# meco-group/omg-tools

Measured on AMD Instinct MI355X. Metric: MPC solves/sec, 1024-agent Holonomic Point2point batch per GPU, higher is better.
Workload: dtype f64

## Files before the change

include/omgx.h:

```cpp
#ifndef OMGX_H
#define OMGX_H
#include <stdint.h>

#ifdef __cplusplus
extern "C" {
#endif

#define OMGX_VERSION 9
#define OMGX_TERM_VARS 4

#define OMGX_OK            0
#define OMGX_E_INVALID    -1
#define OMGX_E_NODEVICE   -2
#define OMGX_E_HIP        -3
#define OMGX_E_TOOLARGE   -4

#define OMGX_SOLVE_SUCCEEDED        0
#define OMGX_MAX_ITER_EXCEEDED      1
#define OMGX_INFEASIBLE_DETECTED    2
#define OMGX_UNSUPPORTED_BOUNDS     3
#define OMGX_NUMERICAL_FAILURE      4

#define OMGX_PTR_DEVICE     1
#define OMGX_BOUNDS_SHARED  2
// ... 71 lines not shown
int  omgx_template_read(const char* path, omgx_template** out);
void omgx_template_free(omgx_template* tpl);

int  omgx_version(void);
const char* omgx_last_error(void);
const char* omgx_status_string(int32_t status);
void omgx_default_options(omgx_options* o);

int  omgx_template_n_blocks(const omgx_template* tpl, int32_t kind);
int  omgx_template_block_at(const omgx_template* tpl, int32_t kind, int32_t i, const char** name, int32_t* off,
                            int32_t* rows, int32_t* cols);
int  omgx_template_block(const omgx_template* tpl, int32_t kind, const char* name, int32_t* off, int32_t* rows,
                         int32_t* cols);

int  omgx_plan_describe(const omgx_template* tpl, omgx_plan_info* info, int32_t* order);

int  omgx_batch_create(const omgx_template* tpl, int32_t n_agents, int32_t device,
                       omgx_batch** out);
void omgx_batch_destroy(omgx_batch* b);
int  omgx_batch_set_options(omgx_batch* b, const omgx_options* o);
int  omgx_batch_set_stream(omgx_batch* b, void* hip_stream);
int  omgx_batch_set_order(omgx_batch* b, const int32_t* order_device);
int  omgx_batch_order_by_iters(omgx_batch* b, const int32_t* iters_device, int32_t* order_device);
int  omgx_batch_set_restarts(omgx_batch* b, const double* x0_alt_device, int32_t n_alt, int32_t* attempts_device);
int  omgx_batch_lds_bytes(const omgx_batch* b);
#define OMGX_HAS_LAST_INSTANCE 1
int  omgx_batch_last_instance(const omgx_batch* b);
int  omgx_batch_workspace(const omgx_batch* b, int32_t* mode, int64_t* lds_bytes,
                          int64_t* hbm_bytes_per_slab, int32_t* n_slabs);

// ... 194 lines not shown
```

omg-tools_amd/csrc/omgx.hip:

```cpp
#include <hip/hip_runtime.h>
#include <hip/hip_ext.h>
#include <cmath>
#include <stdarg.h>
#include <stdio.h>
#include <stdlib.h>
#include <string.h>
#include <string>
#include <vector>
#include "../../include/omgx.h"
#include "omgx_core.h"
#include "omgx_plan.h"
#include "omgx_kernels.h"
#include "omgx_table_cache.h"

namespace {

thread_local std::string g_err;

#define HIPCHK(call)                                                              \
  do {                                                                            \
    hipError_t e_ = (call);                                                       \
    if (e_ != hipSuccess) {                                                       \
      g_err = std::string(#call) + ": " + hipGetErrorString(e_);                  \
      return OMGX_E_HIP;                                                          \
// ... 405 lines not shown
  memset(info, 0, sizeof *info);
  info->n_leaf = d.n_leaf; info->n_root = d.n_root; info->n_eq = d.n_eq; info->nnz_j = d.nnz_j;
  info->kkt_doubles = plan.kkt_doubles; info->wave_path = d.wave_ok;
  info->ws_mode = mode;
  info->lds_bytes = (int64_t)(nl * sizeof(double));
  for (int l = 0; l < d.n_leaf && l < OMGX_PLAN_MAX_LEAF; ++l) {
    info->leaf_size[l] = plan.leaf_off[l + 1] - plan.leaf_off[l];
    info->leaf_bw[l] = plan.leaf_bw[l];
    info->leaf_cpl[l] = plan.cpl_ptr[l + 1] - plan.cpl_ptr[l];
  }
  info->n_pairs = d.n_pairs; info->ka_len = d.ka_len; info->kh_len = d.kh_len; info->kg_len = d.kg_len;
  if (order) for (int q = 0; q < d.N; ++q) order[q] = plan.order[q];
  return OMGX_OK;
}

namespace {
struct TplField { int kind; size_t count; const void* const* src; void** dst; };

size_t tpl_fields(const omgx_template& t, omgx_template* m, TplField* f, int term_vars = OMGX_TERM_VARS) {
  const omgx_template& s = t;
  size_t k = 0;
#define OMGX_F(KD, NAME, CNT) f[k].kind = KD; f[k].count = (size_t)(CNT); f[k].src = (const void* const*)&s.NAME; f[k].dst = m ? (void**)&m->NAME : nullptr; ++k;
  OMGX_F(0, prog, 6 * (size_t)t.n_prog)      OMGX_F(1, knots, t.n_knots)       OMGX_F(0, pp_ptr, t.n_pp + 1)
  OMGX_F(1, pm_coef, t.n_mono)               OMGX_F(0, pm_ptr, t.n_mono + 1)   OMGX_F(0, pm_atom, t.n_matom)
  OMGX_F(0, slot_pp, t.n_slots)              OMGX_F(0, row_ptr, t.n_con + 2)   OMGX_F(1, t_coef, t.n_terms)
  OMGX_F(0, t_slot, t.n_terms)               OMGX_F(0, t_var, (size_t)term_vars * t.n_terms)
  OMGX_F(0, eq_rows, t.n_eq)                 OMGX_F(0, root_vars, t.n_root_vars)
  OMGX_F(2, block_names, t.block_names_len)  OMGX_F(0, block_kind, t.n_blocks)        OMGX_F(0, block_off, t.n_blocks)
  OMGX_F(0, block_rows, t.n_blocks)          OMGX_F(0, block_cols, t.n_blocks)
  OMGX_F(1, lbg_def, t.has_bounds ? t.n_con : 0)  OMGX_F(1, ubg_def, t.has_bounds ? t.n_con : 0)
// ... 1314 lines not shown
```

omg-tools_amd/csrc/omgx_core.h:

```cpp
#pragma once
#include <stdint.h>
#include <math.h>

#ifdef OMGX_HOST_PORT
#define OMGX_FN inline
#define OMGX_HD inline
#define OMGX_HDF inline
#else
#define OMGX_FN __device__ __forceinline__
#define OMGX_HD __host__ __device__ inline
#define OMGX_HDF __host__ __device__ __forceinline__
#endif

#ifdef OMGX_HOST_PORT
#include <vector>
static thread_local std::vector<double> omgx_rbak;
#endif
#ifdef OMGX_COUNT_FACT
#include <atomic>
static std::atomic<long> omgx_dbg_nfact(0);
static std::atomic<long> omgx_dbg_cnt[12];
#endif
namespace omgx {

// ... 18 lines not shown
  int general;
  int rp_packed;
  int n_knots;
  int atoms_alias;
  int wave_ok;
  int n_jv;
  int n_jv4, n_ja4;
  int ka_len, kh_len, kg_len;
  int n_kafix, n_kgfix;
  int n_khfix;
  int side_off, dump_off;
  int n_cs_own;
  int kg_side_dinv;
  int n_owner;
  int n_lift, lift_depth;
};

struct MonoRec { double coef; int16_t a0, a1, a2, a3; };
struct MonoRec8 { double coef; int16_t a0, a1, a2, a3, a4, a5, a6, a7; };

#define OMGX_TV 4
struct JItem { double coef; int16_t slot, va, vb, vc; };
struct RowTerm { double coef; int32_t slot; int16_t v0, v1, v2, v3; };
struct HItem { double coef; int32_t row, target; int16_t slot, vthird, vfourth, kind; };

struct Tables {
  const int32_t* prog; const double* knots;
  const int32_t* pp_ptr; const double* pm_coef; const int32_t* pm_ptr; const int32_t* pm_atom;
  const int32_t* slot_pp;
  const MonoRec* pm_rec;
// ... 301 lines not shown
    if (kHbm) { __builtin_amdgcn_fence(__ATOMIC_RELEASE, "workgroup"); __builtin_amdgcn_wave_barrier(); __builtin_amdgcn_fence(__ATOMIC_ACQUIRE, "workgroup"); }
    else { __builtin_amdgcn_fence(__ATOMIC_RELEASE, "wavefront"); __builtin_amdgcn_wave_barrier(); __builtin_amdgcn_fence(__ATOMIC_ACQUIRE, "wavefront"); }
  }
};
typedef CtxT<false> Ctx;
#endif

#define OMGX_PFOR(i, n) for (int i = c.tid(); i < (n); i += c.nthr())
#define OMGX_PFOR_U4(i, n) _Pragma("unroll 4") for (int i = c.tid(); i < (n); i += c.nthr())

enum { PH_JAC = 0, PH_RESID, PH_ASSEMBLE, PH_FACTOR, PH_SOLVE, PH_STEP, PH_LINESEARCH, PH_UPDATE, PH_F_LEAF, PH_F_SCHUR, PH_F_ROOT, PH_LA, PH_LS, PH_LB, PH_SETUP, PH_TOTAL,
       PH_S_DESC, PH_S_PARAMS, PH_S_JAC0, PH_S_CLASS, PH_S_INIT, PH_A_ZERO, PH_A_PAIRS, PH_A_REST, PH_A_DIAG,
       PH_K_FWD, PH_K_ROOTRHS, PH_K_ROOT, PH_K_LEAFRHS, PH_K_BWD, PH_L_TERMS, PH_L_ROWS,
       PH_F_PARK, PH_F_SWEEP, PH_F_SCALE, PH_A_TCOL, PH_A_HESS, PH_P_LOAD, PH_P_DIV, PH_P_BSPL, PH_P_SLOTS,
       PH_WG_HEAD, PH_WG_TAIL,
       PH_COUNT };
#if defined(OMGX_PROFILE) && !defined(OMGX_HOST_PORT)
#define OMGX_TIC() long long tic_ = (c.sync(), clock64())
#define OMGX_TOC(k) do { c.sync(); long long now_ = clock64(); if (c.tid() == 0 && c.prof) c.prof[k] += now_ - tic_; tic_ = now_; } while (0)
#else
#define OMGX_TIC() do {} while (0)
#define OMGX_TOC(k) do {} while (0)
#endif

OMGX_FN double pp_eval(const Tables& T, int pp, const double* a) {
  double tot = 0.0;
  for (int m = T.pp_ptr[pp]; m < T.pp_ptr[pp + 1]; ++m) {
    double v = T.pm_coef[m];
    for (int q = T.pm_ptr[m]; q < T.pm_ptr[m + 1]; ++q) v *= a[T.pm_atom[q]];
    tot += v;
// ... 698 lines not shown
  Mr.a = ROOT_LDS ? 0 : K.d_off[d.n_leaf]; Mr.ld = 0; Mr.nfact = d.nr; Mr.rows = d.nr + 1; Mr.npos = d.n_root; Mr.dinv = -1; Mr.pan = pan0; Mr.cpl = 0; Mr.bw = d.nr;
  Mr.pad_ = K.d_off[d.n_leaf];
}

template <class C>
OMGX_FN void kkt_describe(const C& c, const Dims& d, const Kkt& K, Work& w, bool sync_after = true) {
  const int who = c.nthr() > 64 ? 64 : 0;
  if (c.tid() == who) kkt_describe_fill<C::wave_only, C::hbm, C::root_lds>(d, K, (BMat*)w.col);
  if (sync_after) c.sync();
}

template <class C>
OMGX_FN void kkt_descriptors(const C& c, const Dims& d, const Tables& T, Work& w, bool sync_after = true) {
  if constexpr (C::wave_only) {
    const int t0 = c.nthr() > 64 ? 64 : 0, nt = c.nthr() > 64 ? 64 : c.nthr();
    const int i0 = c.tid() - t0, n = (d.n_leaf + 1) * (int)(sizeof(BMat) / sizeof(int32_t));
    int32_t* Ms = (int32_t*)w.col;
    if (i0 >= 0 && i0 < nt) for (int i = i0; i < n; i += nt) Ms[i] = T.bmat_img[i];
    if (sync_after) c.sync();
  } else {
    Kkt K; K.bind(d, T, w.kkt);
    kkt_describe(c, d, K, w, sync_after);
  }
}

#ifndef OMGX_HOST_PORT
OMGX_FN WPanel wpanel_leaf(const BMat& M) {
  WPanel P; P.base = M.a; P.ld = M.ld; P.n = M.nfact; P.nreg = M.rows - 2; P.nvec = 2; P.npos = M.nfact; P.bw = M.bw;
  P.vrow = M.rows - 2; P.band = M.bw; P.ldb = M.pad_; P.wbase = M.pan;
  return P;
}
OMGX_FN WPanel wpanel_root(const BMat& M, int n_root) {
  WPanel P; P.base = M.a; P.ld = 0; P.n = M.nfact; P.nreg = M.nfact; P.nvec = 1; P.npos = n_root; P.bw = M.nfact;
  P.vrow = M.nfact; P.band = -1; P.ldb = 0; P.wbase = 0;
  return P;
}

struct DiagLeaf { int base, n, S, dinv, dl; };
OMGX_FN DiagLeaf diag_leaf(const BMat& M) {
  DiagLeaf L;
  L.base = __builtin_amdgcn_readfirstlane(M.a); L.n = __builtin_amdgcn_readfirstlane(M.nfact);
  L.S = __builtin_amdgcn_readfirstlane(M.pan); L.dinv = __builtin_amdgcn_readfirstlane(M.dinv); L.dl = 4 * L.dinv;
  return L;
}

template <class C>
OMGX_FN int kkt_factor_wave(const C& c, const Dims& d, const Kkt& K, Work& w) {
  typedef double v4d __attribute__((ext_vector_type(4)));
  const BMat* Ms = (const BMat*)w.col;
  const int lane = c.lane(), wave = c.wave(), nw = c.nwaves();
  const int koff = (int)(w.kkt - omgx_lds);
  OMGX_TIC();
  int badl = 0;
#ifdef OMGX_PROFILE
  const long long tw0_ = clock64();
#endif
  for (int l = wave; l < d.n_leaf; l += nw) {
    const int kind_bw = __builtin_amdgcn_readfirstlane(Ms[l].bw);
    if (kind_bw < 0) {
      const DiagLeaf L = diag_leaf(Ms[l]);
      const double dj = w.kkt[L.base + (lane < L.n ? lane : 0)];
      if (lane < L.n) { w.dinv[L.dinv + lane] = rcp_pivot(dj); if (!(dj > 0.0)) badl = 1; }
      continue;
    }
    const WPanel P = wpanel_leaf(Ms[l]);
    const int leaf_n = __builtin_amdgcn_readfirstlane(Ms[l].nfact);
    if (wave_leaf_small(leaf_n, kind_bw)) badl |= wave_ldl<OMGX_LEAF_COLS_SMALL, OMGX_LEAF_BW_SMALL, true, 2>(koff, P);
    else badl |= (kind_bw <= 8) ? wave_ldl<OMGX_WAVE_COLS, 8, true, 2>(koff, P) : wave_ldl<OMGX_WAVE_COLS, OMGX_WAVE_COLS, true, 2>(koff, P);
    wave_fence();
    const double dl = wave_dinv<true>(w.kkt, P);
    if (lane < P.n) w.dinv[Ms[l].dinv + lane] = dl;
  }
#ifdef OMGX_PROFILE
  if (c.tid() == 0) { c.prof[PH_F_SCALE] += clock64() - tw0_; c.prof[PH_F_PARK] += 1; }
#endif
  if (c.rmax(badl ? 1.0 : 0.0) > 0.0) return 1;
  OMGX_TOC(PH_F_LEAF);
  double* R = K.R();
  for (int base = 0; base < d.n_leaf; base += nw) {
    const int l = base + wave;
    v4d acc00 = {0.0, 0.0, 0.0, 0.0}, acc10 = acc00, acc11 = acc00;
    int nc1 = 0, ci_b0 = 0, ci_b1 = 0, ci_a[8];
    bool sparse = false;
#pragma unroll
    for (int i = 0; i < 8; ++i) ci_a[i] = 0;
    if (l < d.n_leaf) {
      const BMat M = Ms[l];
      sparse = __builtin_amdgcn_readfirstlane(M.bw) < 0;
      if (!sparse) {
      const int n = __builtin_amdgcn_readfirstlane(M.nfact), ld = __builtin_amdgcn_readfirstlane(M.ld);
      nc1 = __builtin_amdgcn_readfirstlane(M.rows) - n;
      const double* Wt = w.kkt + __builtin_amdgcn_readfirstlane(M.pan);
      const double* di = w.dinv + __builtin_amdgcn_readfirstlane(M.dinv);
      const int32_t* ci = K.cpl_idx + __builtin_amdgcn_readfirstlane(M.cpl);
      const int cb0 = lane & 15, cb1 = 16 + (lane & 15);
      ci_b0 = ci[cb0 < nc1 - 1 ? cb0 : 0]; ci_b1 = ci[cb1 < nc1 - 1 ? cb1 : 0];
#pragma unroll
      for (int i = 0; i < 8; ++i) {
        const int ca = 16 * (i >> 2) + (lane >> 4) + 4 * (i & 3);
        ci_a[i] = ca < nc1 - 1 ? ci[ca] : d.nr;
      }
      const int r0 = lane & 15, r1 = 16 + (lane & 15), q = lane >> 4;
      const int r0c = r0 < nc1 ? r0 : nc1 - 1, r1c = r1 < nc1 ? r1 : nc1 - 1;
      const bool two = nc1 > 16;
      for (int j0 = 0; j0 < n; j0 += 4) {
        const int j = j0 + q, jc = j < n ? j : n - 1;
        const double w0 = Wt[r0c * ld + jc], w1 = Wt[r1c * ld + jc], dj = di[jc];
        const double b0 = (r0 < nc1 && j < n) ? w0 : 0.0, b1 = (r1 < nc1 && j < n) ? w1 : 0.0;
        acc00 = __builtin_amdgcn_mfma_f64_16x16x4f64(b0 * dj, b0, acc00, 0, 0, 0);
        if (two) {
          acc10 = __builtin_amdgcn_mfma_f64_16x16x4f64(b1 * dj, b0, acc10, 0, 0, 0);
          acc11 = __builtin_amdgcn_mfma_f64_16x16x4f64(b1 * dj, b1, acc11, 0, 0, 0);
        }
      }
      }
    }
    const int lend = base + nw < d.n_leaf ? base + nw : d.n_leaf;
    for (int lr = base; lr < lend; ++lr) {
      if (l == lr && !sparse) {
        const int cb0 = lane & 15, cb1 = 16 + (lane & 15);
#pragma unroll
        for (int i = 0; i < 4; ++i) {
          const int ca0 = (lane >> 4) + 4 * i, ca1 = 16 + ca0;
          if (ca0 < nc1 && cb0 < nc1 - 1 && cb0 <= ca0) R[tri(ci_a[i], ci_b0)] -= acc00[i];
          if (ca1 < nc1 && cb0 < nc1 - 1) R[tri(ci_a[4 + i], ci_b0)] -= acc10[i];
          if (ca1 < nc1 && cb1 < nc1 - 1 && cb1 <= ca1) R[tri(ci_a[4 + i], ci_b1)] -= acc11[i];
        }
      } else if (l == lr) {
        const DiagLeaf L = diag_leaf(Ms[l]);
        const int j = lane < L.n ? lane : 0;
        const bool on = lane < L.n;
        const double* A = w.kkt + L.base + j;
        const double di = w.dinv[L.dinv + j];
        const double vt = A[(1 + L.S) * L.n], rj = A[(2 + L.S) * L.n];
        const int pt = d.n_root - 1;
        double vs[4]; int ps[4];
#pragma unroll
        for (int s = 0; s < 4; ++s) {
          const bool has = s < L.S;
          ps[s] = has ? K.dl_pos[L.dl + s * L.n + j] : -1;
          const double v = A[(1 + (has ? s : 0)) * L.n];
          vs[s] = (has && on && ps[s] >= 0) ? v : 0.0;
        }
        if (on) {
#pragma unroll
          for (int s = 0; s < 4; ++s) {
            if (ps[s] < 0 || s >= L.S) continue;
            const double u = vs[s] * di;
#pragma unroll
            for (int s2 = 0; s2 <= s; ++s2) {
              if (ps[s2] < 0) continue;
              const int pa = ps[s] > ps[s2] ? ps[s] : ps[s2], pb = ps[s] > ps[s2] ? ps[s2] : ps[s];
              R[tri(pa, pb)] -= u * vs[s2];
            }
            R[tri(pt, ps[s])] -= u * vt;
            R[tri(d.nr, ps[s])] -= u * rj;
          }
        }
        const double stt = c.wave_sum(on ? vt * di * vt : 0.0), srt = c.wave_sum(on ? rj * di * vt : 0.0);
        if (lane == 0) { R[tri(pt, pt)] -= stt; R[tri(d.nr, pt)] -= srt; }
      }
      c.sync();
    }
  }
  OMGX_TOC(PH_F_SCHUR);
  int badr = 0;
  if (wave == 0) {
    const WPanel P = wpanel_root(Ms[d.n_leaf], d.n_root);
#ifdef OMGX_PROFILE
    const long long tr0_ = clock64();
#endif
    badr = wave_ldl<OMGX_WAVE_COLS, OMGX_WAVE_COLS, false, 1>(koff, P);
#ifdef OMGX_PROFILE
    if (c.tid() == 0) c.prof[PH_F_SWEEP] += clock64() - tr0_;
#endif
  }
  const int bad = c.rmax(badr ? 1.0 : 0.0) > 0.0 ? 2 : 0;
  OMGX_TOC(PH_F_ROOT);
  return bad;
}
// ... 22 lines not shown
    const double y = w.kkt[wcarried<false>(P, P.n) + (lane < P.n ? lane : 0)];
    const double x = wave_bwd<OMGX_WAVE_COLS, false>(koff, P, dl, y * dl);
    if (lane < P.n) sol[d.root_off + lane] = x;
  }
  c.sync();
  OMGX_TOC(PH_K_ROOT);
  double* xg = w.col + OMGX_BMAT_DOUBLES * (OMGX_MAX_LEAF + 1) + wave * 64;
  for (int l = wave; l < d.n_leaf; l += nw) {
    const BMat M = Ms[l];
    if (__builtin_amdgcn_readfirstlane(M.bw) < 0) {
      const DiagLeaf L = diag_leaf(M);
      const int j = lane < L.n ? lane : 0;
      const double* A = w.kkt + L.base + j;
      double acc = A[(2 + L.S) * L.n] - A[(1 + L.S) * L.n] * sol[d.root_off + d.n_root - 1];
      for (int s = 0; s < L.S; ++s) {
        const int ps = K.dl_pos[L.dl + s * L.n + j];
        acc = fma(-A[(1 + s) * L.n], sol[d.root_off + (ps < 0 ? 0 : ps)] * (ps < 0 ? 0.0 : 1.0), acc);
      }
      if (lane < L.n) sol[L.dinv + lane] = acc * w.dinv[L.dinv + j];
      continue;
    }
    const WPanel P = wpanel_uniform(wpanel_leaf(M));
    const int n = P.n, nc = P.nreg + 1 - P.n, ld = P.ld;
    const int32_t* ci = K.cpl_idx + __builtin_amdgcn_readfirstlane(M.cpl);
    if (lane < nc) xg[lane] = sol[d.root_off + ci[lane]];
    wave_fence();
    const int j = lane < n ? lane : 0;
    const double* Wt = w.kkt + P.wbase + j;
    double acc = Wt[nc * ld];
#pragma unroll 4
    for (int a = 0; a < nc; ++a) acc = fma(-Wt[a * ld], xg[a], acc);
    const int dv = __builtin_amdgcn_readfirstlane(M.dinv);
    const double dl = w.dinv[dv + j];
    const double x = wave_leaf_small(n, P.bw) ? wave_bwd<OMGX_LEAF_COLS_SMALL, true>(koff, P, dl, acc * dl)
                                              : wave_bwd<OMGX_WAVE_COLS, true>(koff, P, dl, acc * dl);
    if (lane < n) sol[dv + lane] = x;
    wave_fence();
  }
  c.sync();
  OMGX_TOC(PH_K_BWD);
// ... 23 lines not shown
      wave_fence();
      const int a = lane < nc ? lane : 0;
      double acc = 0.0;
#pragma unroll 4
      for (int q = 0; q < n; ++q) acc = fma(Wt[a * ld + q], xg[q], acc);
      wave_fence();
      if (lane < nc) xg[lane] = acc;
    }
    c.sync();
    if (wave == 0) {
      const int lend = base + nw < d.n_leaf ? base + nw : d.n_leaf;
      for (int lr = base; lr < lend; ++lr) {
        const BMat M = Ms[lr];
        if (__builtin_amdgcn_readfirstlane(M.bw) >= 0) {
          const int nc = __builtin_amdgcn_readfirstlane(M.rows) - 1 - __builtin_amdgcn_readfirstlane(M.nfact);
          const int32_t* ci = K.cpl_idx + __builtin_amdgcn_readfirstlane(M.cpl);
          const double* xs = xg0 + (lr - base) * 64;
          if (lane < nc) R[rrow + ci[lane]] -= xs[lane];
        } else {
          const DiagLeaf L = diag_leaf(M);
          const int j = lane < L.n ? lane : 0;
          const bool on = lane < L.n;
          const double* A = w.kkt + L.base + j;
          const double u = A[(2 + L.S) * L.n] * w.dinv[L.dinv + j];
          for (int s = 0; s < L.S; ++s) {
            const int ps = K.dl_pos[L.dl + s * L.n + j];
            if (on && ps >= 0) R[rrow + ps] -= A[(1 + s) * L.n] * u;
          }
          const double st = c.wave_sum(on ? A[(1 + L.S) * L.n] * u : 0.0);
          if (lane == 0) R[rrow + d.n_root - 1] -= st;
        }
        wave_fence();
      }
    }
    c.sync();
  }
  if (wave == 0) {
    const WPanel P = wpanel_root(Ms[d.n_leaf], d.n_root);
    const double dl = wave_dinv<false>(w.kkt, P);
    const int j = lane < P.n ? lane : 0;
    const double y = wave_fwd_r<false>(koff, P, dl, w.kkt[wcarried<false>(P, P.n) + j]);
    const double x = wave_bwd_r<false>(koff, P, dl, y * dl);
    if (lane < (with_y ? P.n : d.n_root)) out[d.root_off + lane] = x;
  }
  c.sync();
  double* xg = xg0 + wave * 64;
  for (int l = wave; l < d.n_leaf; l += nw) {
    const BMat M = Ms[l];
    if (__builtin_amdgcn_readfirstlane(M.bw) < 0) {
      const DiagLeaf L = diag_leaf(M);
      const int j = lane < L.n ? lane : 0;
      const double* A = w.kkt + L.base + j;
      double acc = A[(2 + L.S) * L.n] - A[(1 + L.S) * L.n] * out[d.root_off + d.n_root - 1];
      for (int s = 0; s < L.S; ++s) {
        const int ps = K.dl_pos[L.dl + s * L.n + j];
        acc = fma(-A[(1 + s) * L.n], out[d.root_off + (ps < 0 ? 0 : ps)] * (ps < 0 ? 0.0 : 1.0), acc);
      }
      if (lane < L.n) out[L.dinv + lane] = acc * w.dinv[L.dinv + j];
      continue;
    }
    const WPanel P = wpanel_uniform(wpanel_leaf(M));
    const int n = P.n, nc = P.nreg + 1 - P.n, ld = P.ld;
    const int32_t* ci = K.cpl_idx + __builtin_amdgcn_readfirstlane(M.cpl);
    if (lane < nc) xg[lane] = out[d.root_off + ci[lane]];
    wave_fence();
    const int j = lane < n ? lane : 0;
    const double* Wt = w.kkt + P.wbase + j;
    double acc = Wt[nc * ld];
#pragma unroll 4
    for (int a = 0; a < nc; ++a) acc = fma(-Wt[a * ld], xg[a], acc);
    const int dv = __builtin_amdgcn_readfirstlane(M.dinv);
    const double dl = w.dinv[dv + j];
    const double x = wave_bwd_r<true>(koff, P, dl, acc * dl);
    if (lane < n) out[dv + lane] = x;
    wave_fence();
  }
  c.sync();
}
#endif
// ... 1309 lines not shown
```

omg-tools_amd/csrc/omgx_plan.h:

```cpp
#pragma once
#include <stdlib.h>
#include <algorithm>
#include <array>
#include <cmath>
#include <map>
#include <functional>
#include <numeric>
#include <queue>
#include <set>
#include <string>
#include <vector>
#include "../../include/omgx.h"
#include "omgx_core.h"

namespace omgx {

struct HostPlan {
  Dims dims;
  Tables tables;
  int kkt_doubles;
  std::vector<int32_t> order, pos, blk, leaf_off, leaf_bw, eq_rows, eq_index;
  std::vector<int32_t> jr_ptr, jr_pos, t_jidx, row_leaf, cpl_ptr, cpl_idx, cpl_map;
  std::vector<int32_t> d_off, b_off;
  std::vector<int32_t> lf_w, lf_ldb, lf_band, lf_kind, dl_pos;
// ... 749 lines not shown
      if (ka_fix.empty()) ka_fix.assign(3, 0);
      if (kg_fix.empty()) kg_fix.assign(3, 0);
      d.side_off = side0;
      d.n_owner = owners;
      kkt_doubles = side0 + n_side + 64;
      d.dump_off = side0 + n_side;
      T.ka_rec = ka_rec.data(); T.kh_rec = kh_rec.data(); T.kg_rec = kg_rec.data();
      T.ka_fix = ka_fix.data(); T.kg_fix = kg_fix.data(); T.kh_fix = kh_fix.data();
    }
    if (pair4.empty()) pair4.assign(4, 0);
    T.pair4 = pair4.data();
    bmat_img.assign(compact ? (size_t)(d.n_leaf + 1) * (sizeof(BMat) / sizeof(int32_t)) : 1, 0);
    if (compact) {
      Kkt K; K.bind(d, T, nullptr);
      kkt_describe_fill<true, false, false>(d, K, (BMat*)bmat_img.data());
    }
    T.bmat_img = bmat_img.data();
    return true;
  }
};

}
```

omg-tools_amd/omgtools/backend.py:

```python
import ctypes as C
import os
import time

import numpy as np


_HERE = os.path.dirname(os.path.abspath(__file__))
LIB_PATH = os.environ.get('OMGX_LIB') or os.path.join(os.path.dirname(_HERE), 'csrc', 'libomgx.so')

PTR_DEVICE, BOUNDS_SHARED, BOUNDS_DEVICE = 1, 2, 4

STATUS_STRINGS = {0: 'Solve_Succeeded', 1: 'Maximum_Iterations_Exceeded',
                  2: 'Infeasible_Problem_Detected', 3: 'Unsupported_Bounds',
                  4: 'Numerical_Failure'}

_I32P, _F64P = C.POINTER(C.c_int32), C.POINTER(C.c_double)


class CTemplate(C.Structure):
    _fields_ = [(n, C.c_int32) for n in
                ('n_var', 'n_par', 'n_con', 'n_atoms', 'n_slots', 'n_terms',
                 'n_prog', 'n_knots', 'n_pp', 'n_mono', 'n_matom')] + \
               [('prog', _I32P), ('knots', _F64P), ('pp_ptr', _I32P), ('pm_coef', _F64P),
                ('pm_ptr', _I32P), ('pm_atom', _I32P), ('slot_pp', _I32P),
# ... 192 lines not shown

def describe_plan(tpl, lib=None):
    lib = lib or load_library()
    ct, keep = make_ctemplate(tpl)
    info = CPlanInfo()
    order = np.zeros(tpl.n_var + 1, dtype=np.int32)
    _check(lib, lib.omgx_plan_describe(C.byref(ct), C.byref(info), order.ctypes.data), 'omgx_plan_describe')
    nl = info.n_leaf
    return dict(n_leaf=nl, n_root=info.n_root, n_eq=info.n_eq, nnz_j=info.nnz_j, kkt_doubles=info.kkt_doubles,
                wave_path=info.wave_path, ws_mode=info.ws_mode, lds_bytes=info.lds_bytes,
                leaf_sizes=list(info.leaf_size[:nl]), leaf_bw=list(info.leaf_bw[:nl]),
                leaf_cpl=list(info.leaf_cpl[:nl]), order=order, n_pairs=info.n_pairs,
                ka_len=info.ka_len, kh_len=info.kh_len, kg_len=info.kg_len)


class AdmmLayoutC(C.Structure):
    _fields_ = [(n, C.c_int32) for n in ('n_dim', 'L', 'n_nghb', 'x_spl', 'p_rel',
                                         'p_zi', 'p_zji', 'p_li', 'p_lji')]


def _ptr(a):
    if a is None:
        return None
    return a.data_ptr() if hasattr(a, 'data_ptr') else (a.ctypes.data if hasattr(a, 'ctypes') else int(a))


def _need(name, a, shape, kind, optional=False):
    if a is None and optional:
        return
    dt = np.dtype(kind.split(' ')[0]) if kind else None
# ... 11 lines not shown
_I, _D, _P, _H = C.c_int32, C.c_double, C.c_void_p, C.c_void_p
_TPL, _LAY, _SIG, _STO = C.POINTER(CTemplate), C.POINTER(AdmmLayoutC), C.POINTER(CSignalsSpec), C.POINTER(CStoreSpec)
_PLA = C.POINTER(CPlantSpec)
PROTOTYPES = {
    'omgx_version': (C.c_int, []),
    'omgx_last_error': (C.c_char_p, []),
    'omgx_status_string': (C.c_char_p, [_I]),
    'omgx_default_options': (None, [C.POINTER(COptions)]),
    'omgx_template_write': (C.c_int, [_TPL, C.c_char_p]),
    'omgx_template_read': (C.c_int, [C.c_char_p, C.POINTER(_TPL)]),
    'omgx_template_free': (None, [_TPL]),
    'omgx_template_n_blocks': (C.c_int, [_TPL, _I]),
    'omgx_template_block_at': (C.c_int, [_TPL, _I, _I, C.POINTER(C.c_char_p), _P, _P, _P]),
    'omgx_template_block': (C.c_int, [_TPL, _I, C.c_char_p, _P, _P, _P]),
    'omgx_plan_describe': (C.c_int, [_TPL, C.POINTER(CPlanInfo), _P]),
    'omgx_batch_create': (C.c_int, [_TPL, _I, _I, C.POINTER(C.c_void_p)]),
    'omgx_batch_destroy': (None, [_H]),
    'omgx_batch_set_options': (C.c_int, [_H, C.POINTER(COptions)]),
    'omgx_batch_set_stream': (C.c_int, [_H, _P]),
    'omgx_batch_set_order': (C.c_int, [_H, _P]),
    'omgx_batch_order_by_iters': (C.c_int, [_H, _P, _P]),
    'omgx_batch_set_restarts': (C.c_int, [_H, _P, _I, _P]),
    'omgx_batch_lds_bytes': (C.c_int, [_H]),
    'omgx_batch_last_instance': (C.c_int, [_H]),
    'omgx_batch_workspace': (C.c_int, [_H, C.POINTER(C.c_int32), C.POINTER(C.c_int64), C.POINTER(C.c_int64), C.POINTER(C.c_int32)]),
    'omgx_batch_solve': (C.c_int, [_H] + [_P] * 8 + [_I]),
    'omgx_batch_sync': (C.c_int, [_H]),
    'omgx_batch_transfer': (C.c_int, [_H, _I, _P, _P, _P]),
    'omgx_batch_eval': (C.c_int, [_H] + [_P] * 7),
    'omgx_batch_set_stats': (C.c_int, [_H, _P, _I]),
# ... 20 lines not shown
    'omgx_batch_predict_measured': (C.c_int, [_H, _P, _P, _D, _D, C.POINTER(CFeedbackSpec)]),
    'omgx_batch_plant_quadrotor_simulate': (C.c_int, [_H, _P, _P, C.POINTER(CQuadPlantSpec), _SIG]),
    'omgx_batch_plant_quadrotor_predict': (C.c_int, [_H, _P, _P, _D, _D, C.POINTER(CQuadPlantSpec), _P, _P, _I]),
    'omgx_batch_obstacles_advance': (C.c_int, [_H, _P, C.POINTER(CObstacleScript), _D, _D]),
    'omgx_batch_set_obstacle_script': (C.c_int, [_H, C.POINTER(CObstacleScript), _P, _I]),
    'omgx_shift_rows': (C.c_int, [_H, _P, _I, _I, _P, _P, _I, _P, _I]),
    'omgx_admm_center': (C.c_int, [_H, _LAY] + [_P] * 3),
    'omgx_admm_update': (C.c_int, [_H, _LAY] + [_P] * 4 + [_D] + [_P] * 4),
    'omgx_admm_update_sums': (C.c_int, [_H, _LAY] + [_P] * 4 + [_D] + [_P] * 5),
    'omgx_admm_communicate': (C.c_int, [_H, _LAY] + [_P] * 5),
    'omgx_admm_center_ex': (C.c_int, [_H, _LAY] + [_P] * 4 + [_I, _P]),
    'omgx_batch_set_center': (C.c_int, [_H, _LAY, _P, _P, _I, _P]),
    'omgx_admm_update_ex': (C.c_int, [_H, _LAY] + [_P] * 4 + [_D] + [_P] * 3 + [_I] + [_P] * 4 + [_I]),
    'omgx_admm_communicate_ex': (C.c_int, [_H, _LAY] + [_P] * 4 + [_I] + [_P] * 2 + [_I, _I, _P]),
}
_NEWER_ENTRIES = ('omgx_batch_set_prepare', 'omgx_batch_set_stop', 'omgx_batch_last_instance')


_lib = None


def load_library(path=None):
    global _lib
    if _lib is not None and path is None:
        return _lib
    path = path or LIB_PATH
    if not os.path.exists(path):
        raise OSError('%s not found: build it with `python __graft_entry__.py` or '
                      '`make -C omg-tools_amd/csrc` (hipcc, gfx950). There is no CPU '
                      'fallback for the solve path.' % path)
    try:
# ... 549 lines not shown
```

Measured before the change: 3.615 million.

## Accumulate Schur complement of identical-coupling leaves in shared MFMA tiles

When every banded leaf couples to the same root columns (at most 32), the planner packs the shared coupling index list and the diagonal leaf's positions into spare descriptor space in LDS. The Schur update then gives each wave a fixed 16x16 tile of the root block and sums all leaves' contributions into it with chained f64 MFMAs. R is loaded and stored once per tile instead of once per leaf, which removes the per-leaf scatter and barrier rounds. The diagonal leaf's update runs in parallel on a fourth wave. The path is gated on template shape and at least three waves, and can be disabled with an environment variable. Profiling counters for the new sub-phases are added.

```diff
diff --git a/include/omgx.h b/include/omgx.h
--- a/include/omgx.h
+++ b/include/omgx.h
@@ -109,6 +109,8 @@
                          int32_t* cols);
 
 int  omgx_plan_describe(const omgx_template* tpl, omgx_plan_info* info, int32_t* order);
+#define OMGX_HAS_SCHUR_TILES 1
+int  omgx_plan_schur_tiles(const omgx_template* tpl, int32_t* n_banded);
 
 int  omgx_batch_create(const omgx_template* tpl, int32_t n_agents, int32_t device,
                        omgx_batch** out);
diff --git a/omg-tools_amd/csrc/omgx.hip b/omg-tools_amd/csrc/omgx.hip
--- a/omg-tools_amd/csrc/omgx.hip
+++ b/omg-tools_amd/csrc/omgx.hip
@@ -443,6 +443,17 @@
   return OMGX_OK;
 }
 
+int omgx_plan_schur_tiles(const omgx_template* tpl, int32_t* n_banded) {
+  if (!n_banded) { g_err = "null argument"; return OMGX_E_INVALID; }
+  TRY(check_template(tpl));
+  omgx::HostPlan plan;
+  size_t nl = 0, ng = 0;
+  int mode = 0, per_cu = 1;
+  if (!plan_for_mode(plan, *tpl, &mode, &nl, &ng, &per_cu)) { g_err = "inconsistent template: " + plan.error; return OMGX_E_INVALID; }
+  *n_banded = plan.dims.schur_tiles;
+  return OMGX_OK;
+}
+
 namespace {
 struct TplField { int kind; size_t count; const void* const* src; void** dst; };
 
diff --git a/omg-tools_amd/csrc/omgx_core.h b/omg-tools_amd/csrc/omgx_core.h
--- a/omg-tools_amd/csrc/omgx_core.h
+++ b/omg-tools_amd/csrc/omgx_core.h
@@ -56,6 +56,7 @@
   int kg_side_dinv;
   int n_owner;
   int n_lift, lift_depth;
+  int schur_tiles, schur_row, schur_dl, schur_ints;
 };
 
 struct MonoRec { double coef; int16_t a0, a1, a2, a3; };
@@ -387,6 +388,7 @@
        PH_K_FWD, PH_K_ROOTRHS, PH_K_ROOT, PH_K_LEAFRHS, PH_K_BWD, PH_L_TERMS, PH_L_ROWS,
        PH_F_PARK, PH_F_SWEEP, PH_F_SCALE, PH_A_TCOL, PH_A_HESS, PH_P_LOAD, PH_P_DIV, PH_P_BSPL, PH_P_SLOTS,
        PH_WG_HEAD, PH_WG_TAIL,
+       PH_F_SCHUR_MFMA, PH_F_SCHUR_SUB,
        PH_COUNT };
 #if defined(OMGX_PROFILE) && !defined(OMGX_HOST_PORT)
 #define OMGX_TIC() long long tic_ = (c.sync(), clock64())
@@ -1115,7 +1117,7 @@
 OMGX_FN void kkt_descriptors(const C& c, const Dims& d, const Tables& T, Work& w, bool sync_after = true) {
   if constexpr (C::wave_only) {
     const int t0 = c.nthr() > 64 ? 64 : 0, nt = c.nthr() > 64 ? 64 : c.nthr();
-    const int i0 = c.tid() - t0, n = (d.n_leaf + 1) * (int)(sizeof(BMat) / sizeof(int32_t));
+    const int i0 = c.tid() - t0, n = d.schur_tiles ? d.schur_ints : (d.n_leaf + 1) * (int)(sizeof(BMat) / sizeof(int32_t));
     int32_t* Ms = (int32_t*)w.col;
     if (i0 >= 0 && i0 < nt) for (int i = i0; i < n; i += nt) Ms[i] = T.bmat_img[i];
     if (sync_after) c.sync();
@@ -1144,42 +1146,154 @@
   L.S = __builtin_amdgcn_readfirstlane(M.pan); L.dinv = __builtin_amdgcn_readfirstlane(M.dinv); L.dl = 4 * L.dinv;
   return L;
 }
+OMGX_FN int diag_leaf_pos(const Dims& d, const Kkt& K, const Work& w, const DiagLeaf& L, int s, int j) {
+  if (d.schur_tiles) return ((const int32_t*)w.col)[d.schur_dl + s * L.n + j];
+  return K.dl_pos[L.dl + s * L.n + j];
+}
+OMGX_FN int leaf_cpl_at(const Dims& d, const Kkt& K, const Work& w, int cpl, int i) {
+  if (d.schur_tiles) return ((const int32_t*)w.col)[d.schur_row + i];
+  return K.cpl_idx[__builtin_amdgcn_readfirstlane(cpl) + i];
+}
+
+struct DiagSchur {
+  double vs[4], di, vt, rj, stt, srt;
+  int ps[4], S;
+  bool on;
+  template <class C>
+  OMGX_FN void load(const C& c, const Dims& d, const Kkt& K, const Work& w, const BMat& M) {
+    const DiagLeaf L = diag_leaf(M);
+    const int lane = c.lane(), j = lane < L.n ? lane : 0;
+    on = lane < L.n; S = L.S;
+    const double* A = w.kkt + L.base + j;
+    di = w.dinv[L.dinv + j];
+    vt = A[(1 + L.S) * L.n]; rj = A[(2 + L.S) * L.n];
+#pragma unroll
+    for (int s = 0; s < 4; ++s) {
+      const bool has = s < L.S;
+      ps[s] = has ? diag_leaf_pos(d, K, w, L, s, j) : -1;
+      const double v = A[(1 + (has ? s : 0)) * L.n];
+      vs[s] = (has && on && ps[s] >= 0) ? v : 0.0;
+    }
+    stt = c.wave_sum(on ? vt * di * vt : 0.0); srt = c.wave_sum(on ? rj * di * vt : 0.0);
+  }
+  template <class C>
+  OMGX_FN void apply(const C& c, const Dims& d, double* R) const {
+    const int pt = d.n_root - 1;
+    if (on) {
+#pragma unroll
+      for (int s = 0; s < 4; ++s) {
+        if (ps[s] < 0 || s >= S) continue;
+        const double u = vs[s] * di;
+#pragma unroll
+        for (int s2 = 0; s2 <= s; ++s2) {
+          if (ps[s2] < 0) continue;
+          const int pa = ps[s] > ps[s2] ? ps[s] : ps[s2], pb = ps[s] > ps[s2] ? ps[s2] : ps[s];
+          R[tri(pa, pb)] -= u * vs[s2];
+        }
+        R[tri(pt, ps[s])] -= u * vt;
+        R[tri(d.nr, ps[s])] -= u * rj;
+      }
+    }
+    if (c.lane() == 0) { R[tri(pt, pt)] -= stt; R[tri(d.nr, pt)] -= srt; }
+  }
+};
+
+template <int CNT>
+OMGX_FN void schur_tile_group(const Work& w, const BMat* Ms, int ra, int cb, int nc1, int q, double (&r)[4]) {
+  typedef double v4d __attribute__((ext_vector_type(4)));
+  const int rac = ra < nc1 ? ra : nc1 - 1, cbc = cb < nc1 ? cb : nc1 - 1;
+  v4d acc[CNT];
+  int n[CNT], ao[CNT], bo[CNT], dv[CNT], nmax = 0, nfull = OMGX_WAVE_ROWS;
+#pragma unroll
+  for (int k = 0; k < CNT; ++k) {
+    const int ld = __builtin_amdgcn_readfirstlane(Ms[k].ld), wo = __builtin_amdgcn_readfirstlane(Ms[k].pan);
+    acc[k] = (v4d){0.0, 0.0, 0.0, 0.0};
+    n[k] = __builtin_amdgcn_readfirstlane(Ms[k].nfact); dv[k] = __builtin_amdgcn_readfirstlane(Ms[k].dinv);
+    ao[k] = wo + rac * ld; bo[k] = wo + cbc * ld;
+    nmax = n[k] > nmax ? n[k] : nmax; nfull = (n[k] & ~3) < nfull ? (n[k] & ~3) : nfull;
+  }
+  double wa[CNT], wb[CNT], dj[CNT];
+  auto request = [&](int j) {
+#pragma unroll
+    for (int k = 0; k < CNT; ++k) {
+      const int jc = j < n[k] ? j : n[k] - 1;
+      wa[k] = w.kkt[ao[k] + jc]; wb[k] = w.kkt[bo[k] + jc]; dj[k] = w.dinv[dv[k] + jc];
+    }
+  };
+  request(q);
+  int j0 = 0;
+  for (; j0 < nfull; j0 += 4) {
+    double a[CNT], b[CNT];
+#pragma unroll
+    for (int k = 0; k < CNT; ++k) { a[k] = wa[k] * dj[k]; b[k] = wb[k]; }
+    request(j0 + 4 + q);
+#pragma unroll
+    for (int k = 0; k < CNT; ++k) acc[k] = __builtin_amdgcn_mfma_f64_16x16x4f64(a[k], b[k], acc[k], 0, 0, 0);
+  }
+  for (; j0 < nmax; j0 += 4) {
+    const int j = j0 + q;
+    double a[CNT], b[CNT];
+#pragma unroll
+    for (int k = 0; k < CNT; ++k) { const bool in = j < n[k]; a[k] = (in ? wa[k] : 0.0) * dj[k]; b[k] = in ? wb[k] : 0.0; }
+    request(j + 4);
+#pragma unroll
+    for (int k = 0; k < CNT; ++k) acc[k] = __builtin_amdgcn_mfma_f64_16x16x4f64(a[k], b[k], acc[k], 0, 0, 0);
+  }
+#pragma unroll
+  for (int k = 0; k < CNT; ++k) {
+#pragma unroll
+    for (int i = 0; i < 4; ++i) r[i] -= acc[k][i];
+  }
+}
 
 template <class C>
-OMGX_FN int kkt_factor_wave(const C& c, const Dims& d, const Kkt& K, Work& w) {
+OMGX_FN void kkt_schur_wave(const C& c, const Dims& d, const Kkt& K, Work& w, [[maybe_unused]] long long ts0_, [[maybe_unused]] long long& tm_) {
   typedef double v4d __attribute__((ext_vector_type(4)));
   const BMat* Ms = (const BMat*)w.col;
   const int lane = c.lane(), wave = c.wave(), nw = c.nwaves();
-  const int koff = (int)(w.kkt - omgx_lds);
-  OMGX_TIC();
-  int badl = 0;
+  double* R = K.R();
+  if (d.schur_tiles && nw >= 3) {
+    const int nb = d.schur_tiles;
+    const int32_t* si = (const int32_t*)w.col + d.schur_row;
+    const int nc1 = __builtin_amdgcn_readfirstlane(Ms[0].rows) - __builtin_amdgcn_readfirstlane(Ms[0].nfact);
+    if (wave == 0 || (wave < 3 && nc1 > 16)) {
+      const int rb = wave >= 1 ? 16 : 0, kb = wave == 2 ? 16 : 0;
+      const int cb = kb + (lane & 15), ci_b = si[cb < nc1 - 1 ? cb : 0];
+      int ad[4]; bool ok[4]; double r[4];
+#pragma unroll
+      for (int i = 0; i < 4; ++i) {
+        const int ca = rb + (lane >> 4) + 4 * i;
+        const int ci_a = ca < nc1 - 1 ? si[ca] : d.nr;
+        ok[i] = ca < nc1 && cb < nc1 - 1 && (rb != kb || cb <= ca);
+        ad[i] = ok[i] ? tri(ci_a, ci_b) : 0;
+      }
+#pragma unroll
+      for (int i = 0; i < 4; ++i) r[i] = R[ad[i]];
+      const int ra = rb + (lane & 15), q = lane >> 4;
+      for (int l0 = 0; l0 < nb; l0 += 3) {
+        const int cnt = nb - l0;
+        if (cnt >= 3) schur_tile_group<3>(w, Ms + l0, ra, cb, nc1, q, r);
+        else if (cnt == 2) schur_tile_group<2>(w, Ms + l0, ra, cb, nc1, q, r);
+        else schur_tile_group<1>(w, Ms + l0, ra, cb, nc1, q, r);
+      }
+#pragma unroll
+      for (int i = 0; i < 4; ++i) if (ok[i]) R[ad[i]] = r[i];
+    }
 #ifdef OMGX_PROFILE
-  const long long tw0_ = clock64();
-#endif
-  for (int l = wave; l < d.n_leaf; l += nw) {
-    const int kind_bw = __builtin_amdgcn_readfirstlane(Ms[l].bw);
-    if (kind_bw < 0) {
-      const DiagLeaf L = diag_leaf(Ms[l]);
-      const double dj = w.kkt[L.base + (lane < L.n ? lane : 0)];
-      if (lane < L.n) { w.dinv[L.dinv + lane] = rcp_pivot(dj); if (!(dj > 0.0)) badl = 1; }
-      continue;
-    }
-    const WPanel P = wpanel_leaf(Ms[l]);
-    const int leaf_n = __builtin_amdgcn_readfirstlane(Ms[l].nfact);
-    if (wave_leaf_small(leaf_n, kind_bw)) badl |= wave_ldl<OMGX_LEAF_COLS_SMALL, OMGX_LEAF_BW_SMALL, true, 2>(koff, P);
-    else badl |= (kind_bw <= 8) ? wave_ldl<OMGX_WAVE_COLS, 8, true, 2>(koff, P) : wave_ldl<OMGX_WAVE_COLS, OMGX_WAVE_COLS, true, 2>(koff, P);
-    wave_fence();
-    const double dl = wave_dinv<true>(w.kkt, P);
-    if (lane < P.n) w.dinv[Ms[l].dinv + lane] = dl;
-  }
+    tm_ = clock64() - ts0_;
+#endif
+    const int dw = nw > 3 ? 3 : 0;
+    const bool diag = nb < d.n_leaf && wave == dw;
+    DiagSchur D;
+    if (diag) D.load(c, d, K, w, Ms[nb]);
+    c.sync();
+    if (diag) D.apply(c, d, R);
+    c.sync();
+  } else for (int base = 0; base < d.n_leaf; base += nw) {
+    const int l = base + wave;
 #ifdef OMGX_PROFILE
-  if (c.tid() == 0) { c.prof[PH_F_SCALE] += clock64() - tw0_; c.prof[PH_F_PARK] += 1; }
-#endif
-  if (c.rmax(badl ? 1.0 : 0.0) > 0.0) return 1;
-  OMGX_TOC(PH_F_LEAF);
-  double* R = K.R();
-  for (int base = 0; base < d.n_leaf; base += nw) {
-    const int l = base + wave;
+    const long long tb_ = clock64();
+#endif
     v4d acc00 = {0.0, 0.0, 0.0, 0.0}, acc10 = acc00, acc11 = acc00;
     int nc1 = 0, ci_b0 = 0, ci_b1 = 0, ci_a[8];
     bool sparse = false;
@@ -1193,13 +1307,12 @@
       nc1 = __builtin_amdgcn_readfirstlane(M.rows) - n;
       const double* Wt = w.kkt + __builtin_amdgcn_readfirstlane(M.pan);
       const double* di = w.dinv + __builtin_amdgcn_readfirstlane(M.dinv);
-      const int32_t* ci = K.cpl_idx + __builtin_amdgcn_readfirstlane(M.cpl);
       const int cb0 = lane & 15, cb1 = 16 + (lane & 15);
-      ci_b0 = ci[cb0 < nc1 - 1 ? cb0 : 0]; ci_b1 = ci[cb1 < nc1 - 1 ? cb1 : 0];
+      ci_b0 = leaf_cpl_at(d, K, w, M.cpl, cb0 < nc1 - 1 ? cb0 : 0); ci_b1 = leaf_cpl_at(d, K, w, M.cpl, cb1 < nc1 - 1 ? cb1 : 0);
 #pragma unroll
       for (int i = 0; i < 8; ++i) {
         const int ca = 16 * (i >> 2) + (lane >> 4) + 4 * (i & 3);
-        ci_a[i] = ca < nc1 - 1 ? ci[ca] : d.nr;
+        ci_a[i] = ca < nc1 - 1 ? leaf_cpl_at(d, K, w, M.cpl, ca) : d.nr;
       }
       const int r0 = lane & 15, r1 = 16 + (lane & 15), q = lane >> 4;
       const int r0c = r0 < nc1 ? r0 : nc1 - 1, r1c = r1 < nc1 ? r1 : nc1 - 1;
@@ -1216,6 +1329,9 @@
       }
       }
     }
+#ifdef OMGX_PROFILE
+    tm_ += clock64() - tb_;
+#endif
     const int lend = base + nw < d.n_leaf ? base + nw : d.n_leaf;
     for (int lr = base; lr < lend; ++lr) {
       if (l == lr && !sparse) {
@@ -1228,43 +1344,55 @@
           if (ca1 < nc1 && cb1 < nc1 - 1 && cb1 <= ca1) R[tri(ci_a[4 + i], ci_b1)] -= acc11[i];
         }
       } else if (l == lr) {
-        const DiagLeaf L = diag_leaf(Ms[l]);
-        const int j = lane < L.n ? lane : 0;
-        const bool on = lane < L.n;
-        const double* A = w.kkt + L.base + j;
-        const double di = w.dinv[L.dinv + j];
-        const double vt = A[(1 + L.S) * L.n], rj = A[(2 + L.S) * L.n];
-        const int pt = d.n_root - 1;
-        double vs[4]; int ps[4];
-#pragma unroll
-        for (int s = 0; s < 4; ++s) {
-          const bool has = s < L.S;
-          ps[s] = has ? K.dl_pos[L.dl + s * L.n + j] : -1;
-          const double v = A[(1 + (has ? s : 0)) * L.n];
-          vs[s] = (has && on && ps[s] >= 0) ? v : 0.0;
-        }
-        if (on) {
-#pragma unroll
-          for (int s = 0; s < 4; ++s) {
-            if (ps[s] < 0 || s >= L.S) continue;
-            const double u = vs[s] * di;
-#pragma unroll
-            for (int s2 = 0; s2 <= s; ++s2) {
-              if (ps[s2] < 0) continue;
-              const int pa = ps[s] > ps[s2] ? ps[s] : ps[s2], pb = ps[s] > ps[s2] ? ps[s2] : ps[s];
-              R[tri(pa, pb)] -= u * vs[s2];
-            }
-            R[tri(pt, ps[s])] -= u * vt;
-            R[tri(d.nr, ps[s])] -= u * rj;
-          }
-        }
-        const double stt = c.wave_sum(on ? vt * di * vt : 0.0), srt = c.wave_sum(on ? rj * di * vt : 0.0);
-        if (lane == 0) { R[tri(pt, pt)] -= stt; R[tri(d.nr, pt)] -= srt; }
+        DiagSchur D;
+        D.load(c, d, K, w, Ms[l]);
+        D.apply(c, d, R);
       }
       c.sync();
     }
   }
+}
+
+template <class C>
+OMGX_FN int kkt_factor_wave(const C& c, const Dims& d, const Kkt& K, Work& w) {
+  const BMat* Ms = (const BMat*)w.col;
+  const int lane = c.lane(), wave = c.wave(), nw = c.nwaves();
+  const int koff = (int)(w.kkt - omgx_lds);
+  OMGX_TIC();
+  int badl = 0;
+#ifdef OMGX_PROFILE
+  const long long tw0_ = clock64();
+#endif
+  for (int l = wave; l < d.n_leaf; l += nw) {
+    const int kind_bw = __builtin_amdgcn_readfirstlane(Ms[l].bw);
+    if (kind_bw < 0) {
+      const DiagLeaf L = diag_leaf(Ms[l]);
+      const double dj = w.kkt[L.base + (lane < L.n ? lane : 0)];
+      if (lane < L.n) { w.dinv[L.dinv + lane] = rcp_pivot(dj); if (!(dj > 0.0)) badl = 1; }
+      continue;
+    }
+    const WPanel P = wpanel_leaf(Ms[l]);
+    const int leaf_n = __builtin_amdgcn_readfirstlane(Ms[l].nfact);
+    if (wave_leaf_small(leaf_n, kind_bw)) badl |= wave_ldl<OMGX_LEAF_COLS_SMALL, OMGX_LEAF_BW_SMALL, true, 2>(koff, P);
+    else badl |= (kind_bw <= 8) ? wave_ldl<OMGX_WAVE_COLS, 8, true, 2>(koff, P) : wave_ldl<OMGX_WAVE_COLS, OMGX_WAVE_COLS, true, 2>(koff, P);
+    wave_fence();
+    const double dl = wave_dinv<true>(w.kkt, P);
+    if (lane < P.n) w.dinv[Ms[l].dinv + lane] = dl;
+  }
+#ifdef OMGX_PROFILE
+  if (c.tid() == 0) { c.prof[PH_F_SCALE] += clock64() - tw0_; c.prof[PH_F_PARK] += 1; }
+#endif
+  if (c.rmax(badl ? 1.0 : 0.0) > 0.0) return 1;
+  OMGX_TOC(PH_F_LEAF);
+  [[maybe_unused]] long long ts0_ = 0, tm_ = 0;
+#ifdef OMGX_PROFILE
+  ts0_ = clock64();
+#endif
+  kkt_schur_wave(c, d, K, w, ts0_, tm_);
   OMGX_TOC(PH_F_SCHUR);
+#ifdef OMGX_PROFILE
+  if (c.tid() == 0) { c.prof[PH_F_SCHUR_MFMA] += tm_; c.prof[PH_F_SCHUR_SUB] += tic_ - ts0_ - tm_; }
+#endif
   int badr = 0;
   if (wave == 0) {
     const WPanel P = wpanel_root(Ms[d.n_leaf], d.n_root);
@@ -1317,7 +1445,7 @@
       const double* A = w.kkt + L.base + j;
       double acc = A[(2 + L.S) * L.n] - A[(1 + L.S) * L.n] * sol[d.root_off + d.n_root - 1];
       for (int s = 0; s < L.S; ++s) {
-        const int ps = K.dl_pos[L.dl + s * L.n + j];
+        const int ps = diag_leaf_pos(d, K, w, L, s, j);
         acc = fma(-A[(1 + s) * L.n], sol[d.root_off + (ps < 0 ? 0 : ps)] * (ps < 0 ? 0.0 : 1.0), acc);
       }
       if (lane < L.n) sol[L.dinv + lane] = acc * w.dinv[L.dinv + j];
@@ -1325,8 +1453,7 @@
     }
     const WPanel P = wpanel_uniform(wpanel_leaf(M));
     const int n = P.n, nc = P.nreg + 1 - P.n, ld = P.ld;
-    const int32_t* ci = K.cpl_idx + __builtin_amdgcn_readfirstlane(M.cpl);
-    if (lane < nc) xg[lane] = sol[d.root_off + ci[lane]];
+    if (lane < nc) xg[lane] = sol[d.root_off + leaf_cpl_at(d, K, w, M.cpl, lane)];
     wave_fence();
     const int j = lane < n ? lane : 0;
     const double* Wt = w.kkt + P.wbase + j;
@@ -1380,9 +1507,8 @@
         const BMat M = Ms[lr];
         if (__builtin_amdgcn_readfirstlane(M.bw) >= 0) {
           const int nc = __builtin_amdgcn_readfirstlane(M.rows) - 1 - __builtin_amdgcn_readfirstlane(M.nfact);
-          const int32_t* ci = K.cpl_idx + __builtin_amdgcn_readfirstlane(M.cpl);
           const double* xs = xg0 + (lr - base) * 64;
-          if (lane < nc) R[rrow + ci[lane]] -= xs[lane];
+          if (lane < nc) R[rrow + leaf_cpl_at(d, K, w, M.cpl, lane)] -= xs[lane];
         } else {
           const DiagLeaf L = diag_leaf(M);
           const int j = lane < L.n ? lane : 0;
@@ -1390,7 +1516,7 @@
           const double* A = w.kkt + L.base + j;
           const double u = A[(2 + L.S) * L.n] * w.dinv[L.dinv + j];
           for (int s = 0; s < L.S; ++s) {
-            const int ps = K.dl_pos[L.dl + s * L.n + j];
+            const int ps = diag_leaf_pos(d, K, w, L, s, j);
             if (on && ps >= 0) R[rrow + ps] -= A[(1 + s) * L.n] * u;
           }
           const double st = c.wave_sum(on ? A[(1 + L.S) * L.n] * u : 0.0);
@@ -1419,7 +1545,7 @@
       const double* A = w.kkt + L.base + j;
       double acc = A[(2 + L.S) * L.n] - A[(1 + L.S) * L.n] * out[d.root_off + d.n_root - 1];
       for (int s = 0; s < L.S; ++s) {
-        const int ps = K.dl_pos[L.dl + s * L.n + j];
+        const int ps = diag_leaf_pos(d, K, w, L, s, j);
         acc = fma(-A[(1 + s) * L.n], out[d.root_off + (ps < 0 ? 0 : ps)] * (ps < 0 ? 0.0 : 1.0), acc);
       }
       if (lane < L.n) out[L.dinv + lane] = acc * w.dinv[L.dinv + j];
@@ -1427,8 +1553,7 @@
     }
     const WPanel P = wpanel_uniform(wpanel_leaf(M));
     const int n = P.n, nc = P.nreg + 1 - P.n, ld = P.ld;
-    const int32_t* ci = K.cpl_idx + __builtin_amdgcn_readfirstlane(M.cpl);
-    if (lane < nc) xg[lane] = out[d.root_off + ci[lane]];
+    if (lane < nc) xg[lane] = out[d.root_off + leaf_cpl_at(d, K, w, M.cpl, lane)];
     wave_fence();
     const int j = lane < n ? lane : 0;
     const double* Wt = w.kkt + P.wbase + j;
diff --git a/omg-tools_amd/csrc/omgx_plan.h b/omg-tools_amd/csrc/omgx_plan.h
--- a/omg-tools_amd/csrc/omgx_plan.h
+++ b/omg-tools_amd/csrc/omgx_plan.h
@@ -787,10 +787,34 @@
     if (compact) {
       Kkt K; K.bind(d, T, nullptr);
       kkt_describe_fill<true, false, false>(d, K, (BMat*)bmat_img.data());
+      const int nb = schur_rule();
+      if (nb > 0) {
+        d.schur_tiles = nb; d.schur_row = (int)bmat_img.size();
+        bmat_img.insert(bmat_img.end(), cpl_idx.begin() + cpl_ptr[0], cpl_idx.begin() + cpl_ptr[1]);
+        d.schur_dl = (int)bmat_img.size();
+        if (nb < d.n_leaf) bmat_img.insert(bmat_img.end(), dl_pos.begin() + 4 * (size_t)leaf_off[nb], dl_pos.begin() + 4 * (size_t)leaf_off[nb] + (size_t)lf_w[nb] * (leaf_off[nb + 1] - leaf_off[nb]));
+        d.schur_ints = (int)bmat_img.size();
+      }
     }
     T.bmat_img = bmat_img.data();
     return true;
   }
+
+  int schur_rule() const {
+    const Dims& d = dims;
+    if (!compact || !d.wave_ok || d.n_leaf < 1 || owners / 64 < 3 || getenv("OMGX_NO_SCHUR_TILES")) return 0;
+    int nb = 0;
+    while (nb < d.n_leaf && !lf_kind[nb]) ++nb;
+    if (nb == 0 || d.n_leaf - nb > 1) return 0;
+    for (int l = nb; l < d.n_leaf; ++l) if (!lf_kind[l]) return 0;
+    const int nc = cpl_ptr[1] - cpl_ptr[0];
+    if (nc + 1 > 32) return 0;
+    for (int l = 1; l < nb; ++l)
+      if (cpl_ptr[l + 1] - cpl_ptr[l] != nc || !std::equal(cpl_idx.begin() + cpl_ptr[l], cpl_idx.begin() + cpl_ptr[l + 1], cpl_idx.begin())) return 0;
+    const int dl_ints = nb < d.n_leaf ? lf_w[nb] * (leaf_off[nb + 1] - leaf_off[nb]) : 0;
+    const int free_ints = (OMGX_MAX_LEAF - d.n_leaf) * (int)(sizeof(BMat) / sizeof(int32_t));
+    return nc + dl_ints <= free_ints ? nb : 0;
+  }
 };
 
 }
diff --git a/omg-tools_amd/omgtools/backend.py b/omg-tools_amd/omgtools/backend.py
--- a/omg-tools_amd/omgtools/backend.py
+++ b/omg-tools_amd/omgtools/backend.py
@@ -230,6 +230,14 @@
                 ka_len=info.ka_len, kh_len=info.kh_len, kg_len=info.kg_len)
 
 
+def plan_schur_tiles(tpl, lib=None):
+    lib = lib or load_library()
+    ct, keep = make_ctemplate(tpl)
+    n = C.c_int32(-1)
+    _check(lib, lib.omgx_plan_schur_tiles(C.byref(ct), C.byref(n)), 'omgx_plan_schur_tiles')
+    return int(n.value)
+
+
 class AdmmLayoutC(C.Structure):
     _fields_ = [(n, C.c_int32) for n in ('n_dim', 'L', 'n_nghb', 'x_spl', 'p_rel',
                                          'p_zi', 'p_zji', 'p_li', 'p_lji')]
@@ -271,6 +279,7 @@
     'omgx_template_block_at': (C.c_int, [_TPL, _I, _I, C.POINTER(C.c_char_p), _P, _P, _P]),
     'omgx_template_block': (C.c_int, [_TPL, _I, C.c_char_p, _P, _P, _P]),
     'omgx_plan_describe': (C.c_int, [_TPL, C.POINTER(CPlanInfo), _P]),
+    'omgx_plan_schur_tiles': (C.c_int, [_TPL, _P]),
     'omgx_batch_create': (C.c_int, [_TPL, _I, _I, C.POINTER(C.c_void_p)]),
     'omgx_batch_destroy': (None, [_H]),
     'omgx_batch_set_options': (C.c_int, [_H, C.POINTER(COptions)]),
@@ -321,7 +330,7 @@
     'omgx_admm_update_ex': (C.c_int, [_H, _LAY] + [_P] * 4 + [_D] + [_P] * 3 + [_I] + [_P] * 4 + [_I]),
     'omgx_admm_communicate_ex': (C.c_int, [_H, _LAY] + [_P] * 4 + [_I] + [_P] * 2 + [_I, _I, _P]),
 }
-_NEWER_ENTRIES = ('omgx_batch_set_prepare', 'omgx_batch_set_stop', 'omgx_batch_last_instance')
+_NEWER_ENTRIES = ('omgx_batch_set_prepare', 'omgx_batch_set_stop', 'omgx_batch_last_instance', 'omgx_plan_schur_tiles')
 
 
 _lib = None
```

Result: faster. 3.674 million, median of 6 (+1.6%).
